# google-research/semivl

Measured on AMD Instinct MI355X. Metric: train images/sec (512^2, ViT-B/16), higher is better.
Workload: dtype f32 (fp32 in / out / accumulate everywhere; the MFMA products as split 16-bit terms with fp32 accumulation: the ViT's linears, in_proj weight gradients and fused attention and the decoder's 3x3 convolutions (tiled: forward, input and weight gradient; dilated: forward, input gradient) on fp16 x 2 ope; 1 GPU; SemiVL step, pascal N=21, vlm-vlg-aspp-s2p4-sk04-ftap-mcvitb, 512x512, bs=16/GPU labeled + 16/GPU unlabeled (BASELINE configs[1]); global_batch=32, parallelism=dp1

## Files before the change

### include/semivl_hip.h

```cpp
#ifndef SEMIVL_HIP_H_
#define SEMIVL_HIP_H_

#include <stddef.h>
#include <stdint.h>

#ifdef __cplusplus
extern "C" {
#endif

typedef void* svl_stream_t;

typedef enum svl_status {
  SVL_OK = 0,
  SVL_ERR_INVALID_ARG = -1,
  SVL_ERR_LAUNCH = -2,
  SVL_ERR_UNSUPPORTED = -3
} svl_status;

int svl_version(void);
int svl_stream_release(svl_stream_t stream);
int svl_stream_prepare(svl_stream_t stream);
int svl_stream_helper(svl_stream_t stream, void** helper);
int svl_shutdown(void);
int svl_num_stream_contexts(void);
// ... 94 lines not shown
  int64_t p_rows;
  const float* bias;
  int act;
  float* preact;
  const float* resid;
  int64_t ldr;
  int accumulate;
  int fmt;
  int p_fmt;
  const int32_t* a_sexp;
  const int32_t* b_sexp;
  const float* a_rnorm;
  const float* b_bound;
  int32_t* p_sexp;
} svl_pgemm_desc;
int64_t svl_planes_rows(int64_t rows);
int64_t svl_planes_bytes(int64_t rows, int K);
int svl_split_planes_bf16x3(const float* x, int64_t ld, int64_t k_stride, int64_t rows, int K, void* planes,
                            int64_t planes_rows, int64_t row_off, svl_stream_t stream);
int64_t svl_planes_bytes_fmt(int64_t rows, int K, int fmt);
int svl_split_planes_f16x2(const float* x, int64_t ld, int64_t k_stride, int64_t rows, int K, void* planes,
                           int64_t planes_rows, int64_t row_off, int32_t* sexp, float* rnorm, unsigned* tensor_amax,
                           svl_stream_t stream);
int svl_gemm_planes_f32(const svl_pgemm_desc* d, svl_stream_t stream);
int svl_conv3x3_wgrad_tiled_groups(int imgs, int H, int W, int Ct, int Co);
int svl_conv3x3_wgrad_tiled(const float* dy, int64_t lddy, int Co, const float* src1, int64_t ld1, int C1,
                            const float* src2, int64_t ld2, int C2, int rep, int imgs, int H, int W, float* slabs,
                            int groups, const float* gn_in, svl_stream_t stream);

int svl_reduce_slabs_f32(float* out, const float* slabs, int nslab, int64_t count, int accumulate,
                         svl_stream_t stream);


int svl_softmax_max_f32(const float* logits, int B, int N, int64_t HW, float* conf, int64_t* label,
                        svl_stream_t stream);

int svl_cutmix_f32(float* out, const float* a, const float* b, const float* box, int B, int C, int64_t HW,
                   svl_stream_t stream);
int svl_cutmix_i64(int64_t* out, const int64_t* a, const int64_t* b, const float* box, int B, int64_t HW,
                   svl_stream_t stream);

typedef struct svl_ce_desc {
  const float* logits;
  int B, N;
  int64_t HW;
  const int64_t* target;
// ... 85 lines not shown
int svl_layernorm_bwd(const float* dy, const float* x, const float* stats, const float* gamma, int64_t rows,
                      int C, const float* dx_add, float* dx, float* dgamma_part, float* dbeta_part,
                      svl_stream_t stream);
int svl_softmax_rows_fwd(float* s, int64_t rows, int cols, int64_t ld, float scale, svl_stream_t stream);
int svl_softmax_rows_bwd(float* dp, const float* p, int64_t rows, int cols, int64_t ld, float scale,
                         svl_stream_t stream);

int svl_l2norm_fwd(const float* x, int64_t rows, int C, float eps, float* y, float* inv_norm, svl_stream_t stream);
int svl_l2norm_bwd(const float* dy, const float* y, const float* inv_norm, int64_t rows, int C, float* dx,
                   svl_stream_t stream);

int64_t svl_colsum_ws_floats(int64_t rows, int C);
int svl_colsum_f32(const float* x, int64_t rows, int C, int64_t ld, float* out, int accumulate, float* ws,
                   svl_stream_t stream);

int svl_eltwise_f32(int mode, const float* a, const float* b, float* out, int64_t n, svl_stream_t stream);
int svl_chanmask_f32(const float* x, const float* mask, float scale, int64_t rows, int rows_per_img, int C,
                     float* out, svl_stream_t stream);
int svl_fill_f32(float* p, float v, int64_t n, svl_stream_t stream);
int svl_bernoulli_f32(float* p, int64_t n, float keep_prob, uint64_t seed, uint64_t offset, svl_stream_t stream);
int svl_affine_planes_f32(const float* x, int64_t planes, int C, int64_t HW, const float* k4, float* y, svl_stream_t stream);
int svl_copy2d_f32(const float* src, int64_t sgrp, int64_t src_go, int64_t src_ld, float* dst, int64_t dgrp,
                   int64_t dst_go, int64_t dst_ld, int64_t rows, int C, int accumulate, svl_stream_t stream);
int svl_permute4_f32(const float* src, float* dst, int64_t n0, int64_t n1, int64_t n2, int64_t n3, int64_t s0, int64_t s1,
                     int64_t s2, int64_t s3, svl_stream_t stream);
int svl_bound2_f32(const float* rnorm, int64_t rows, const float* bias, int64_t nbias, float* out2, svl_stream_t stream);
int svl_permute_rows_f32(const float* src, int64_t outer, int A, int B, int C, float* dst, svl_stream_t stream);

int svl_groupnorm_fwd(const float* x, int64_t ldx, const float* gamma, const float* beta, float eps, int imgs,
                      int64_t HW, int C, int G, int relu, float* y, int64_t ldy, float* stats, svl_stream_t stream);
int64_t svl_conv3x3_gn_ws_doubles(int imgs, int H, int W, int N);
int svl_conv3x3_gn_f32(const float* src1, int64_t ld1, int C1, const float* src2, int64_t ld2, int C2, int rep,
                       const float* w, int imgs, int H, int W, int N, float* out, int64_t ldo, float eps, double* ws,
                       float* stats, const float* gn_in, const void* w_planes, svl_stream_t stream);
int64_t svl_conv3x3_weight_planes_bytes(int N, int Ct);
int svl_conv3x3_weight_planes(const float* w, int N, int Ct, void* planes, svl_stream_t stream);
int svl_groupnorm_scale_shift(const float* stats, const float* gamma, const float* beta, int imgs, int C, int G, float* scsh,
                              svl_stream_t stream);
int svl_groupnorm_apply(const float* x, int64_t ldx, const float* gamma, const float* beta, int imgs, int64_t HW, int C, int G,
                        int relu, const float* stats, float* y, int64_t ldy, svl_stream_t stream);
int svl_groupnorm_bwd(const float* dy, int64_t lddy, const float* x, int64_t ldx, const float* y, int64_t ldy,
                      const float* stats, const float* gamma, const float* beta, int imgs, int64_t HW, int C, int G,
                      int relu, float* dx, int64_t lddx, float* chan_sums, svl_stream_t stream);
int64_t svl_conv3x3_gnb_ws_doubles(int imgs, int H, int W, int N);
int svl_conv3x3_dgrad_gnb_f32(const float* dy, int64_t lddy, int C1, const float* w, int imgs, int H, int W, int N, float* out,
                              int64_t ldo, int accumulate, const float* gnb_x, const float* gnb_table, const float* gnb_stats,
// ... 126 lines not shown
```

### semivl_amd/csrc/api.hip

```cpp
#include "svl_common.h"
#include <stdarg.h>

#include <map>
#include <mutex>
#include <utility>

static thread_local char g_err[512] = {0};

void svl_set_error(const char* fmt, ...) {
  va_list ap;
  va_start(ap, fmt);
  vsnprintf(g_err, sizeof(g_err), fmt, ap);
  va_end(ap);
}

extern "C" int svl_version(void) { return 604; }

extern "C" int svl_last_error(char* buf, size_t len) {
  const size_t n = strlen(g_err);
  if (buf && len > 0) {
    const size_t c = n < len - 1 ? n : len - 1;
    memcpy(buf, g_err, c);
    buf[c] = 0;
  }
  return (int)n;
}

namespace {
struct StreamCtx {
  hipStream_t aux = nullptr;
  hipEvent_t fork = nullptr, join = nullptr;
};
std::mutex g_mu;
std::map<std::pair<int, hipStream_t>, StreamCtx> g_ctx;

int stream_device(hipStream_t st, int* dev) {
  if (hipGetDevice(dev) != hipSuccess) {
    svl_set_error("hipGetDevice failed");
    return SVL_ERR_LAUNCH;
// ... 111 lines not shown
```

### semivl_amd/csrc/gemm_planes_h2.hip

```cpp
#include "gemm_planes_impl.h"
#include <stdlib.h>

int svl_planes_launch_h2(const PlanesP& p, hipStream_t st) { return launch<2>(p, st); }

namespace {

__global__ __launch_bounds__(256) void pack_planes_h2_kernel(const float* __restrict__ x, long ld, long ks, long rows, int K,
                                                             char* __restrict__ planes, long p_ks, long row_off,
                                                             int* __restrict__ sexp, float* __restrict__ rnorm,
                                                             unsigned* __restrict__ tensor_amax) {
  __shared__ float s_max[8][32];
  __shared__ double s_sq[8][32];
  __shared__ int s_e[32];
  const int tid = threadIdx.x;
  const long rb = blockIdx.x;
  const bool rowmajor = ks == 1;
  const bool fast = rowmajor && (ld & 3) == 0 && ((reinterpret_cast<uintptr_t>(x) & 15) == 0) && (K & 3) == 0;
  if (rowmajor) {
    const int row = tid >> 3, sub = tid & 7;
    const long r = rb * 32 + row;
    float amax = 0.f;
    double sq = 0.0;
    if (r < rows) {
      const float* src = x + r * ld;
      if (fast) {
        for (int k = sub * 4; k < K; k += 32) {
          const float4 f = *reinterpret_cast<const float4*>(src + k);
          amax = fmaxf(fmaxf(amax, fabsf(f.x)), fmaxf(fabsf(f.y), fmaxf(fabsf(f.z), fabsf(f.w))));
          sq += (double)f.x * f.x + (double)f.y * f.y + ((double)f.z * f.z + (double)f.w * f.w);
        }
      } else {
        for (int k = sub; k < K; k += 8) {
          const float f = src[k];
          amax = fmaxf(amax, fabsf(f));
          sq += (double)f * f;
        }
      }
    }
// ... 9 lines not shown
    float amax = 0.f;
    double sq = 0.0;
    if (r < rows)
      for (int k = part; k < K; k += 8) {
        const float f = x[r * ld + (long)k * ks];
        amax = fmaxf(amax, fabsf(f));
        sq += (double)f * f;
      }
    s_max[part][r31] = amax;
    s_sq[part][r31] = sq;
  }
  __syncthreads();
  if (tid < 32) {
    float amax = s_max[0][tid];
    double sq = s_sq[0][tid];
    if (!rowmajor)
      for (int q = 1; q < 8; ++q) { amax = fmaxf(amax, s_max[q][tid]); sq += s_sq[q][tid]; }
    const long r = rb * 32 + tid;
    const int e = r < rows ? scale_exp_of(amax) : 0;
    s_e[tid] = e;
    const long rr = row_off + rb * 32 + tid;
    sexp[rr] = e;
    if (rnorm) rnorm[rr] = r < rows ? (float)(sqrt(sq) * (1.0 + 1e-6)) : 0.f;
    if (tensor_amax && blockIdx.y == 0) {
      float m = r < rows ? amax : 0.f;
#pragma unroll
      for (int o = 16; o > 0; o >>= 1) m = fmaxf(m, __shfl_xor(m, o, 64));
      if (tid == 0 && m > 0.f) atomicMax(tensor_amax, __float_as_uint(m));
    }
  }
  __syncthreads();
  const int nkg = K >> 4;
  const int kg_lo = (int)((long)nkg * blockIdx.y / gridDim.y), kg_hi = (int)((long)nkg * (blockIdx.y + 1) / gridDim.y);
  for (int idx = kg_lo * 64 + tid; idx < kg_hi * 64; idx += 256) {
    const int r31 = idx & 31, h = (idx >> 5) & 1, kg = idx >> 6;
    const long r = rb * 32 + r31;
    float v[8];
    if (r < rows) {
      const float* src = x + r * ld + (long)(kg * 16 + 4 * h) * ks;
      if (fast) {
        const float4 f0 = *reinterpret_cast<const float4*>(src), f1 = *reinterpret_cast<const float4*>(src + 8);
        v[0] = f0.x; v[1] = f0.y; v[2] = f0.z; v[3] = f0.w; v[4] = f1.x; v[5] = f1.y; v[6] = f1.z; v[7] = f1.w;
      } else {
#pragma unroll
        for (int q = 0; q < 4; ++q) { v[q] = src[q * ks]; v[4 + q] = src[(8 + q) * ks]; }
      }
    } else {
#pragma unroll
      for (int q = 0; q < 8; ++q) v[q] = 0.f;
    }
    f16x8 h0, h1;
    split2x8(v, s_e[r31], h0, h1);
    const long rr = row_off + r;
    char* q = planes + (long)kg * p_ks + (rr >> 5) * (2 * CH) + (h * 32 + (int)(rr & 31)) * 16;
    *reinterpret_cast<f16x8*>(q) = h0;
    *reinterpret_cast<f16x8*>(q + CH) = h1;
  }
}

}

extern "C" int svl_split_planes_f16x2(const float* x, int64_t ld, int64_t k_stride, int64_t rows, int K, void* planes,
                                      int64_t planes_rows, int64_t row_off, int32_t* sexp, float* rnorm, unsigned* tensor_amax,
                                      svl_stream_t stream) {
  SVL_CHECK_ARG(x && planes && sexp && rows > 0 && K > 0 && (K & 15) == 0 && k_stride >= 1 && planes_rows >= row_off + rows &&
                    row_off >= 0 && (planes_rows & 255) == 0 && (row_off & 31) == 0,
                "svl_split_planes_f16x2: bad args (K %% 16, planes_rows %% 256, row_off %% 32 must be 0; sexp required)");
  const long blocks = (rows + 31) / 32;
  int ysplit = 1;
  if (blocks < 256) {
    ysplit = (int)(512 / blocks);
    if (ysplit > 8) ysplit = 8;
    if (ysplit > (K >> 6)) ysplit = K >> 6;
    if (ysplit < 1) ysplit = 1;
  }
  if (tensor_amax) SVL_HIP_CHECK(hipMemsetAsync(tensor_amax, 0, 4, (hipStream_t)stream));
  hipLaunchKernelGGL(pack_planes_h2_kernel, dim3((unsigned)blocks, (unsigned)ysplit), dim3(256), 0, (hipStream_t)stream, x, (long)ld,
                     (long)k_stride, (long)rows, K, (char*)planes, (long)planes_rows * 64, (long)row_off, sexp, rnorm, tensor_amax);
  SVL_LAUNCH_CHECK("svl_split_planes_f16x2");
  return SVL_OK;
}
```

### semivl_amd/csrc/norm.hip

```cpp
#include "svl_common.h"
#include "planes_split_h2.h"

namespace {

inline int grid_for(long n, int per_thread = 1) {
  long g = (n + 256L * per_thread - 1) / (256L * per_thread);
  if (g < 1) g = 1;
  if (g > 256 * 16) g = 256 * 16;
  return (int)g;
}

__device__ __forceinline__ void ln_emit_planes(const float* __restrict__ src, long r0, long rows, int C,
                                               const float* __restrict__ gamma, const float* __restrict__ beta,
                                               const float* st , char* __restrict__ planes, long p_ks) {
  const int t = threadIdx.x, r31 = t & 31, h = (t >> 5) & 1, kg0 = t >> 6;
  const long r = r0 + r31;
  const int nkg = C >> 4;
  float mean = 0.f, rstd = 0.f;
  mean = st[2 * r31]; rstd = st[2 * r31 + 1];
  for (int kg = kg0; kg < nkg; kg += 4) {
    float v[8];
    const int k = kg * 16 + 4 * h;
    if (r < rows) {
      const float4 f0 = *reinterpret_cast<const float4*>(src + r * C + k), f1 = *reinterpret_cast<const float4*>(src + r * C + k + 8);
// ... 414 lines not shown
  }
}
__global__ void chanmask_kernel(const float* __restrict__ x, const float* __restrict__ mask, float scale, long rows,
                                int rows_per_img, int C, float* __restrict__ out) {
  const long n = rows * C;
  for (long i = (long)blockIdx.x * blockDim.x + threadIdx.x; i < n; i += (long)gridDim.x * blockDim.x) {
    const long r = i / C;
    const int c = (int)(i - r * C);
    out[i] = x[i] * mask[(r / rows_per_img) * C + c] * scale;
  }
}
__global__ void copy2d_kernel(const float* __restrict__ src, long sgrp, long src_go, long src_ld,
                              float* __restrict__ dst, long dgrp, long dst_go, long dst_ld, long rows, int C,
                              int accumulate) {
  const long n = rows * C;
  for (long t = (long)blockIdx.x * blockDim.x + threadIdx.x; t < n; t += (long)gridDim.x * blockDim.x) {
    const long i = t / C;
    const int c = (int)(t - i * C);
    const float v = src[(i / sgrp) * src_go + (i % sgrp) * src_ld + c];
    float* d = dst + (i / dgrp) * dst_go + (i % dgrp) * dst_ld + c;
    *d = accumulate ? (*d + v) : v;
  }
}
__global__ void affine_planes_kernel(const float* __restrict__ x, long planes, int C, long HW, const float* __restrict__ k,
                                     float* __restrict__ y) {
  const long n = planes * HW;
  for (long i = (long)blockIdx.x * blockDim.x + threadIdx.x; i < n; i += (long)gridDim.x * blockDim.x) {
    const int c = (int)((i / HW) % C);
    y[i] = ((x[i] * k[c] + k[C + c]) - k[2 * C + c]) / k[3 * C + c];
  }
}
__global__ void bernoulli_kernel(float* p, long n, float keep, unsigned long long seed, unsigned long long offset) {
  for (long i = (long)blockIdx.x * blockDim.x + threadIdx.x; i < n; i += (long)gridDim.x * blockDim.x) {
    unsigned long long z = seed + (offset + (unsigned long long)i + 1ull) * 0x9E3779B97F4A7C15ull;
    z = (z ^ (z >> 30)) * 0xBF58476D1CE4E5B9ull;
    z = (z ^ (z >> 27)) * 0x94D049BB133111EBull;
    z ^= z >> 31;
    const float u = (float)(z >> 40) * (1.0f / 16777216.0f);
    p[i] = u < keep ? 1.f : 0.f;
  }
}
__global__ void fill_kernel(float* p, float v, long n) {
  for (long i = (long)blockIdx.x * blockDim.x + threadIdx.x; i < n; i += (long)gridDim.x * blockDim.x) p[i] = v;
}

template <int NT>
// ... 780 lines not shown
  const long total = (long)(n0 * n1 * n2 * n3);
  hipLaunchKernelGGL(permute4_kernel, dim3(grid_for(total, 4)), dim3(256), 0, (hipStream_t)stream, src, dst, (long)n1, (long)n2,
                     (long)n3, (long)s0, (long)s1, (long)s2, (long)s3, total);
  SVL_LAUNCH_CHECK("svl_permute4_f32");
  return SVL_OK;
}

extern "C" int svl_bound2_f32(const float* rnorm, int64_t rows, const float* bias, int64_t nbias, float* out2,
                              svl_stream_t stream) {
  SVL_CHECK_ARG(rnorm && rows > 0 && out2 && (!bias || nbias > 0), "svl_bound2_f32: bad args");
  hipLaunchKernelGGL(bound2_kernel, dim3(1), dim3(256), 0, (hipStream_t)stream, rnorm, (long)rows, bias, (long)nbias, out2);
  SVL_LAUNCH_CHECK("svl_bound2_f32");
  return SVL_OK;
}

extern "C" int svl_copy2d_f32(const float* src, int64_t sgrp, int64_t src_go, int64_t src_ld, float* dst, int64_t dgrp,
                              int64_t dst_go, int64_t dst_ld, int64_t rows, int C, int accumulate, svl_stream_t stream) {
  SVL_CHECK_ARG(src && dst && sgrp >= 1 && dgrp >= 1 && rows > 0 && C > 0, "svl_copy2d_f32: bad args");
  hipLaunchKernelGGL(copy2d_kernel, dim3(grid_for(rows * C, 4)), dim3(256), 0, (hipStream_t)stream, src, (long)sgrp,
                     (long)src_go, (long)src_ld, dst, (long)dgrp, (long)dst_go, (long)dst_ld, (long)rows, C, accumulate);
  SVL_LAUNCH_CHECK("svl_copy2d_f32");
  return SVL_OK;
}
```

### semivl_amd/lib.py

```python
import ctypes as C
import os
import subprocess

import torch

_HERE = os.path.dirname(os.path.abspath(__file__))
LIB_PATH = os.path.join(_HERE, "libsemivl_hip.so")
CSRC = os.path.join(_HERE, "csrc")

c_f32p = C.c_void_p
c_i64p = C.c_void_p


class Operand(C.Structure):
    _fields_ = [("ptr", C.c_void_p), ("ld", C.c_int64), ("bs_outer", C.c_int64), ("bs_inner", C.c_int64)]


class ConvGeom(C.Structure):
    _fields_ = [("H", C.c_int), ("W", C.c_int), ("Ho", C.c_int), ("Wo", C.c_int), ("stride", C.c_int),
                ("C1", C.c_int), ("C2", C.c_int), ("rep", C.c_int),
                ("KH", C.c_int), ("KW", C.c_int), ("dil", C.c_int), ("pad", C.c_int), ("sign", C.c_int),
                ("src2", C.c_void_p), ("ld2", C.c_int64), ("patch", C.c_int)]


# ... 24 lines not shown

class CeDesc(C.Structure):
    _fields_ = [("logits", C.c_void_p), ("B", C.c_int), ("N", C.c_int), ("HW", C.c_int64),
                ("target", C.c_void_p), ("use_ignore_t", C.c_int), ("conf", C.c_void_p), ("ign", C.c_void_p),
                ("conf_thresh", C.c_float), ("all_pixels", C.c_int), ("mc_target", C.c_void_p), ("partials", C.c_void_p),
                ("dlogits", C.c_void_p), ("gscale", C.c_void_p), ("img_weight", C.c_void_p)]


class CeUpDesc(C.Structure):
    _fields_ = [("logits", C.c_void_p), ("B", C.c_int), ("N", C.c_int), ("h", C.c_int), ("w", C.c_int), ("H", C.c_int),
                ("W", C.c_int), ("align_corners", C.c_int), ("target", C.c_void_p), ("use_ignore_t", C.c_int),
                ("conf", C.c_void_p), ("ign", C.c_void_p), ("conf_thresh", C.c_float), ("all_pixels", C.c_int),
                ("mc_target", C.c_void_p), ("partials", C.c_void_p), ("dlogits", C.c_void_p), ("gscale", C.c_void_p),
                ("img_weight", C.c_void_p)]


class SeqAttnDesc(C.Structure):
    _fields_ = [("groups", C.c_int), ("inner", C.c_int), ("seq", C.c_int), ("heads", C.c_int),
                ("outer_stride", C.c_int64), ("inner_stride", C.c_int64), ("seq_stride", C.c_int64),
                ("qkv", C.c_void_p), ("out", C.c_void_p), ("probs", C.c_void_p),
                ("dout", C.c_void_p), ("dqkv", C.c_void_p), ("dscores", C.c_void_p)]


_I, _L, _F, _D, _P = C.c_int, C.c_int64, C.c_float, C.c_double, C.c_void_p
SIGNATURES = {
    "svl_version": (_I, []),
    "svl_last_error": (_I, [C.c_char_p, C.c_size_t]),
    "svl_gemm_f32": (_I, [C.POINTER(GemmDesc), _P]),
    "svl_set_gemm_emulation": (_I, [_I]),
    "svl_get_gemm_emulation": (_I, []),
    "svl_set_conv_tiled": (_I, [_I]),
    "svl_planes_rows": (_L, [_L]),
    "svl_planes_bytes": (_L, [_L, _I]),
    "svl_split_planes_bf16x3": (_I, [_P, _L, _L, _L, _I, _P, _L, _L, _P]),
    "svl_planes_bytes_fmt": (_L, [_L, _I, _I]),
    "svl_split_planes_f16x2": (_I, [_P, _L, _L, _L, _I, _P, _L, _L, _P, _P, _P, _P]),
    "svl_gemm_planes_f32": (_I, [C.POINTER(PGemmDesc), _P]),
    "svl_conv3x3_wgrad_tiled_groups": (_I, [_I, _I, _I, _I, _I]),
    "svl_conv3x3_wgrad_tiled": (_I, [_P, _L, _I, _P, _L, _I, _P, _L, _I, _I, _I, _I, _I, _P, _I, _P, _P]),
    "svl_reduce_slabs_f32": (_I, [_P, _P, _I, _L, _I, _P]),
    "svl_softmax_max_f32": (_I, [_P, _I, _I, _L, _P, _P, _P]),
    "svl_cutmix_f32": (_I, [_P, _P, _P, _P, _I, _I, _L, _P]),
    "svl_cutmix_i64": (_I, [_P, _P, _P, _P, _I, _L, _P]),
    "svl_ce_num_blocks": (_L, [_I, _I, _L]),
    "svl_ce_fused_f32": (_I, [C.POINTER(CeDesc), _P]),
    "svl_ce_finalize": (_I, [_P, _L, _P, _P]),
    "svl_ce_up_num_blocks": (_L, [_I, _I, _I, _I, _I, _I, _I]),
    "svl_ce_up_fused_f32": (_I, [C.POINTER(CeUpDesc), _P]),
    "svl_softmax_max_up_f32": (_I, [_P, _I, _I, _I, _I, _I, _I, _I, _P, _P, _P]),
    "svl_semivl_gscale": (_I, [_P, _D, _F, _P, _P, _P, _P]),
    "svl_semivl_loss": (_I, [_P, _D, _F, _P, _P, _P, _P]),
    "svl_inv_count_f32": (_I, [_P, _P, _P]),
    "svl_conf_ratio_f32": (_I, [_P, _P, _I, _L, _F, _P, _P, _P]),
    "svl_conf_avg_ws_doubles": (_L, [_I]),
    "svl_conf_avg_factor": (_I, [_P, _P, _I, _L, _P, _P, _P]),
    "svl_stream_release": (_I, [_P]),
    "svl_stream_prepare": (_I, [_P]),
    "svl_stream_helper": (_I, [_P, C.POINTER(C.c_void_p)]),
    "svl_last_gemm_path": (_I, []),
# ... 13 lines not shown
    "svl_concept_max_f32": (_I, [_P, _I, _I, _L, _P, _I, _P, _P]),
    "svl_iou_hist_i64": (_I, [_P, _P, _L, _I, _I, _P, _P]),
    "svl_layernorm_fwd": (_I, [_P, _P, _P, _F, _L, _I, _P, _P, _P]),
    "svl_layernorm_fwd_planes": (_I, [_P, _P, _P, _F, _L, _I, _P, _P, _P, _L, _P]),
    "svl_layernorm_fwd_planes_f16x2": (_I, [_P, _P, _P, _F, _L, _I, _P, _P, _P, _L, _P, _P, _P]),
    "svl_layernorm_fwd_pack_f16x2": (_I, [_P, _P, _P, _F, _L, _I, _P, _P, _P, _L, _L, _P, _P, _I, _P, _P]),
    "svl_layernorm_bwd_pack_f16x2": (_I, [_P, _P, _P, _P, _L, _I, _P, _P, _P, _L, _L, _P, _P, _P, _P]),
    "svl_layernorm_bwd_parts": (_I, [_L]),
    "svl_layernorm_bwd": (_I, [_P, _P, _P, _P, _L, _I, _P, _P, _P, _P, _P]),
    "svl_softmax_rows_fwd": (_I, [_P, _L, _I, _L, _F, _P]),
    "svl_softmax_rows_bwd": (_I, [_P, _P, _L, _I, _L, _F, _P]),
    "svl_l2norm_fwd": (_I, [_P, _L, _I, _F, _P, _P, _P]),
    "svl_l2norm_bwd": (_I, [_P, _P, _P, _L, _I, _P, _P]),
    "svl_colsum_ws_floats": (_L, [_L, _I]),
    "svl_colsum_f32": (_I, [_P, _L, _I, _L, _P, _I, _P, _P]),
    "svl_eltwise_f32": (_I, [_I, _P, _P, _P, _L, _P]),
    "svl_chanmask_f32": (_I, [_P, _P, _F, _L, _I, _I, _P, _P]),
    "svl_fill_f32": (_I, [_P, _F, _L, _P]),
    "svl_affine_planes_f32": (_I, [_P, _L, _I, _L, _P, _P, _P]),
    "svl_permute_rows_f32": (_I, [_P, _L, _I, _I, _I, _P, _P]),
    "svl_permute4_f32": (_I, [_P, _P, _L, _L, _L, _L, _L, _L, _L, _L, _P]),
    "svl_bound2_f32": (_I, [_P, _L, _P, _L, _P, _P]),
    "svl_copy2d_f32": (_I, [_P, _L, _L, _L, _P, _L, _L, _L, _L, _I, _I, _P]),
    "svl_groupnorm_fwd": (_I, [_P, _L, _P, _P, _F, _I, _L, _I, _I, _I, _P, _L, _P, _P]),
    "svl_conv3x3_gn_ws_doubles": (_L, [_I, _I, _I, _I]),
    "svl_conv3x3_gn_f32": (_I, [_P, _L, _I, _P, _L, _I, _I, _P, _I, _I, _I, _I, _P, _L, _F, _P, _P, _P, _P, _P]),
    "svl_conv3x3_weight_planes_bytes": (_L, [_I, _I]),
    "svl_conv3x3_weight_planes": (_I, [_P, _I, _I, _P, _P]),
    "svl_groupnorm_scale_shift": (_I, [_P, _P, _P, _I, _I, _I, _P, _P]),
    "svl_groupnorm_apply": (_I, [_P, _L, _P, _P, _I, _L, _I, _I, _I, _P, _P, _L, _P]),
    "svl_groupnorm_bwd": (_I, [_P, _L, _P, _L, _P, _L, _P, _P, _P, _I, _L, _I, _I, _I, _P, _L, _P, _P]),
    "svl_conv3x3_gnb_ws_doubles": (_L, [_I, _I, _I, _I]),
    "svl_conv3x3_dgrad_gnb_f32": (_I, [_P, _L, _I, _P, _I, _I, _I, _I, _P, _L, _I, _P, _P, _P, _P, _P, _P, _P]),
    "svl_groupnorm_bwd_apply": (_I, [_P, _L, _P, _L, _P, _P, _P, _I, _L, _I, _I, _I, _P, _P, _L, _P]),
    "svl_bn_ws_doubles": (_L, [_L, _I]),
    "svl_bn_stats": (_I, [_P, _L, _L, _I, _P, _P, _P]),
    "svl_bn_finalize": (_I, [_P, _D, _F, _F, _P, _P, _I, _P, _P, _P]),
    "svl_bn_eval_invstd": (_I, [_P, _F, _I, _P, _P]),
    "svl_bn_apply": (_I, [_P, _L, _L, _I, _P, _P, _P, _P, _P, _L, _I, _P, _L, _P]),
    "svl_bn_bwd_reduce": (_I, [_P, _L, _P, _L, _P, _L, _P, _P, _P, _P, _L, _I, _P, _P, _P]),
    "svl_bn_bwd_apply": (_I, [_P, _L, _P, _L, _P, _L, _P, _P, _P, _P, _P, _D, _L, _I, _P, _L, _P, _L, _P]),
    "svl_maxpool3x3s2_fwd": (_I, [_P, _I, _I, _I, _I, _P, _P, _P]),
    "svl_maxpool3x3s2_bwd": (_I, [_P, _P, _I, _I, _I, _I, _P, _P]),
    "svl_aug_resample_u8": (_I, [_P, _I, _I, _I, _I, _I, _I, _I, _I, _I, _I, _I, _I, _P, _P]),
    "svl_aug_to_float": (_I, [_P, _I, C.POINTER(C.c_float), C.POINTER(C.c_float), _P, _P]),
    "svl_aug_mask_i64": (_I, [_P, _I, _I, _I, _P, _P]),
# ... 78 lines not shown
```

### semivl_amd/model/vit.py

```python
import math

import torch
import torch.nn as nn
import torch.nn.functional as F

from .. import gradsync, ops


class _MHAParams(nn.Module):
    def __init__(self, dims):
        super().__init__()
        self.in_proj_weight = nn.Parameter(torch.empty(3 * dims, dims))
        self.in_proj_bias = nn.Parameter(torch.zeros(3 * dims))
        self.out_proj = nn.Linear(dims, dims)
        nn.init.xavier_uniform_(self.in_proj_weight)
        nn.init.constant_(self.out_proj.bias, 0.)


class _AttnParams(nn.Module):
    def __init__(self, dims):
        super().__init__()
        self.attn = _MHAParams(dims)


# ... 180 lines not shown
        if dp.get("attn") is not None:
            dbr = ops.droppath_scale(dx2, dp["attn"], dp["keep"], Bn, T)
            dbrp = ops.split_planes(dbr) if pp else None
        do = ops.matmul_nn(dbrp if dbrp is not None else dbr, p["wout"])
        wout_parts.append((dbr, s["o"]))
        if D == 64 and pp and ops.attention_planes_ok() and not (s["want_v"] and dv is not None):
            dqkv, dqkv_p = ops.attention_bwd(do, s["qkv"], s["o"], s["P"], Bn, T, heads, planes=True, sets=s.get("sets"))
            dqkv_amax = dqkv_p.amax
        elif D == 64:
            dqkv = ops.attention_bwd(do, s["qkv"], s["o"], s["P"], Bn, T, heads, sets=s.get("sets"))
        else:
            dqkv = ops.vit_attention_bwd(do, s["qkv"], s["P"], Bn, T, heads, D)
        dx_res = dx2
    dvproj = None
    if s["want_v"] and dv is not None:
        dvo, dvop = ffn_ln_bwd(dv, None, s["vo"], s["st2v"], s["hv_pre"], dp.get("ffn_v"))
        dvproj = ops.matmul_nn(dvop if dvop is not None else dvo, p["wout"])
        wout_parts.append((dvo, s["vproj"]))
        dx_res = dvo if dx_res is None else ops.add(dx_res, dvo)
    if dqkv is not None and dvproj is not None:
        rows = dqkv.shape[0]
        ops.copy2d(dvproj, 0, rows, 0, E, dqkv, 2 * E, rows, 0, 3 * E, rows, E, accumulate=True)
        dvproj = dqkv_amax = None
    g["wout_parts"] = wout_parts
    if dqkv is not None:
        g["in_full"] = (dqkv, y1, dqkv_amax, s.get("y1_amax"))
        dy1 = ops.matmul_nn(dqkv_p if dqkv_p is not None else dqkv, p["win"])
    elif dvproj is not None:
        g["in_v"] = (dvproj, y1)
        dy1 = ops.matmul_nn(dvproj, p["win"][2 * E:])
    else:
        return dx_res, None, g
    if "ln1w" in want or "ln1b" in want:
        r_ = ops.layernorm_bwd(dy1, x, s["st1"], p["ln1w"], dx_add=dx_res, want_wgrad=True, planes=pp)
        g["ln1w"], g["ln1b"] = [("add", r_[1])], [("add", r_[2])]
        return r_[0], (r_[3] if pp else None), g
    if pp:
        dx_in, dx_in_p = ops.layernorm_bwd(dy1, x, s["st1"], p["ln1w"], dx_add=dx_res, planes=True)
        return dx_in, dx_in_p, g
    return ops.layernorm_bwd(dy1, x, s["st1"], p["ln1w"], dx_add=dx_res), None, g


def ffn_ln_wgrads(p, g):
    out = {}
    for key, parts in g.items():
        if key not in FFN_LN_KEYS:
# ... 554 lines not shown
            if bias.requires_grad:
                grads[id(bias)] = sink_grad(bias, lambda dst, acc: ops.colsum(df, out=dst, accumulate=acc))
        rest = [q for q in ctx.params if q is m.pos_embed or not any(q is r_ for l_ in m.layers for r_ in l_.parameters())]
        if dx is None:
            gradsync.ready(rest)
            ctx.saved = None
            return (None, None, None, None) + tuple(grads.get(id(p)) for p in ctx.params)
        if m.ln0.weight.requires_grad or m.ln0.bias.requires_grad:
            dxpre, dg_, db_ = ops.layernorm_bwd(dx, s["x_pre"], s["st0"], m.ln0.weight, want_wgrad=True)
            _sink_vectors(grads, ((m.ln0.weight, dg_), (m.ln0.bias, db_)))
        else:
            dxpre = ops.layernorm_bwd(dx, s["x_pre"], s["st0"], m.ln0.weight)
        if m.cls_token.requires_grad:
            grads[id(m.cls_token)] = sink_grad(m.cls_token, lambda dst, acc: ops.colsum(
                dxpre.view(B, T * E), out=dst.view(-1), accumulate=acc, C_=E, ld=T * E))
        wpe = m.patch_embed.projection.weight
        if wpe.requires_grad:
            dtok = ops.empty(B * NP, E, device=dev)
            ops.copy2d(dxpre, E, NP, T * E, E, dtok, 0, NP, NP * E, E, B * NP, E)
            img = s["img"]
            grads[id(wpe)] = sink_grad(wpe, lambda dst, acc: ops.matmul_tn_patch(
                dtok, img, m.patch_size, out=dst.view(E, -1), accumulate=acc))
        def pos_fn(dst, acc):
            ops.copy2d(dxpre, 0, B * T, 0, E, dst.view(-1), 0, T, 0, E, T, E, accumulate=acc)
            for b in range(1, B):
                ops.copy2d(dxpre, b * T * E, T, 0, E, dst.view(-1), 0, T, 0, E, T, E, accumulate=True)
        dpos_in = None
        if ctx.pos_is_input:
            if m.pos_embed.requires_grad:
                dpos_in = ops.empty(T, E, device=dev)
                pos_fn(dpos_in, False)
        elif m.pos_embed.requires_grad:
            grads[id(m.pos_embed)] = sink_grad(m.pos_embed, pos_fn)
        gradsync.ready(rest)
        ctx.saved = None
        return (None, None, None, dpos_in) + tuple(grads.get(id(p)) for p in ctx.params)
```

### semivl_amd/ops.py

```python
import collections
import ctypes as C
import os
import math
import weakref

import torch

from . import lib as L

A_KC, A_MC, A_CONV, A_PATCH = 0, 1, 2, 3
B_KC, B_NC, B_CONVW = 0, 1, 2
B_NC_GELU, B_NC_LN, B_PATCHT = 3, 4, 5
ACT_NONE, ACT_GELU, ACT_RELU, ACT_MUL_DGELU, ACT_MUL_DRELU = 0, 1, 2, 3, 4
OUT_STRIDED, OUT_CONVT2X, OUT_PATCH = 0, 1, 2


def _st():
    return C.c_void_p(torch.cuda.current_stream().cuda_stream)


PROFILE = None
PROFILE_SCOPE = None


# ... 231 lines not shown
        main.wait_event(ev)
        q, seq = _WG_KEEP.get(main.device.index), getattr(ev, "_svl_seq", -1)
        while q and q[0][2] <= seq:
            q.popleft()
        return
    wg = _WG.get(main.device.index)
    if wg is not None and wg.cuda_stream != main.cuda_stream:
        main.wait_stream(wg)
        _WG_KEEP[main.device.index].clear()
        for t in produced:
            if isinstance(t, torch.Tensor) and t.is_cuda:
                t.record_stream(main)


def planes_rows(rows):
    return (rows + 255) // 256 * 256


PLANES_FMT = os.environ.get("SVL_PLANES_FMT", "h2")
assert PLANES_FMT in ("h2", "b3")


class Planes:
    __slots__ = ("buf", "rows", "K", "prow", "fmt", "sexp", "rnorm", "amax", "_bd")

    def __init__(self, rows, K, device=None, buf=None, fmt=None, sexp=None, rnorm=None):
        assert K % 16 == 0
        self.fmt = fmt or PLANES_FMT
        self.rows, self.K, self.prow = rows, K, planes_rows(rows)
        dev = device if device is not None else (buf.device if buf is not None else torch.cuda.current_device())
        self._bd = self.amax = None
        if self.fmt == "h2":
            self.buf = buf if buf is not None else torch.empty(K // 16 * self.prow * 32, dtype=torch.float16, device=dev)
            self.sexp = sexp if sexp is not None else torch.empty(self.prow, dtype=torch.int32, device=dev)
            self.rnorm = rnorm
        else:
            self.buf = buf if buf is not None else torch.empty(K // 16 * self.prow * 48, dtype=torch.bfloat16, device=dev)
            self.sexp = self.rnorm = None

    @property
    def shape(self):
        return (self.rows, self.K)

    def kslice(self, k0, k1):
        assert k0 % 16 == 0 and k1 % 16 == 0 and 0 <= k0 < k1 <= self.K
        per = self.prow * (32 if self.fmt == "h2" else 48)
        return Planes(self.rows, k1 - k0, buf=self.buf[k0 // 16 * per:k1 // 16 * per], fmt=self.fmt, sexp=self.sexp,
                      rnorm=self.rnorm)


ONEPASS = not os.environ.get("SVL_NO_ONEPASS")


def split_planes(x2d, out=None, row_off=0, transpose=False, fmt=None, want_amax=False):
    assert x2d.dim() == 2 and x2d.dtype == torch.float32
    if transpose:
        K, rows = x2d.shape
        assert x2d.stride(1) == 1
        ld, ks = 1, x2d.stride(0)
    else:
        rows, K = x2d.shape
        assert x2d.stride(1) == 1
        ld, ks = x2d.stride(0), 1
    if out is None:
        out = Planes(rows, K, device=x2d.device, fmt=fmt)
# ... 36 lines not shown
        elif hasattr(v, "buf"):
            yield v.buf
            for extra in (getattr(v, "sexp", None), getattr(v, "rnorm", None)):
                if extra is not None:
                    yield extra

    def get(self):
        if self.ev is not None:
            s = torch.cuda.current_stream()
            if s.cuda_stream not in self.seen:
                s.wait_event(self.ev)
                for t in self._tensors(self.val):
                    if t.is_cuda:
                        t.record_stream(s)
                self.seen.add(s.cuda_stream)
        return self.val


def weights_changed():
    global WEIGHT_EPOCH
    WEIGHT_EPOCH += 1


def weight_planes(W, transpose=False, fmt=None):
    fmt = fmt or PLANES_FMT

    def build():
        return split_planes(W.detach(), transpose=transpose, fmt=fmt)

    base = W._base if W._base is not None else W
    if not isinstance(base, torch.nn.Parameter):
        return build()
    key = (W.data_ptr(), tuple(W.shape), W.stride(0), transpose, fmt)
    ver = (base._version, WEIGHT_EPOCH if base.requires_grad else 0)
    hit = _WPLANES.get(key)
    if hit is not None and hit[0] == ver and hit[2]() is base:
        return hit[1].get()
    pl = build()
    if len(_WPLANES) > 4096:
        _WPLANES.clear()
    _WPLANES[key] = (ver, StreamCached(pl), weakref.ref(base))
    return pl


def _out_bound(B, bias):
    key = (None if bias is None else (bias.data_ptr(), bias._version, WEIGHT_EPOCH if bias.requires_grad else 0),
           torch.cuda.current_stream().cuda_stream)
    if B._bd is None:
        B._bd = {}
    hit = B._bd.get(key)
    if hit is not None:
        return hit
    bd = torch.empty(2, dtype=torch.float32, device=B.buf.device)
    bflat = bias.detach().view(-1) if bias is not None else None
    L.check(L.load().svl_bound2_f32(_p(B.rnorm), B.rows, _p(bflat), bflat.numel() if bflat is not None else 0, _p(bd), _st()),
            "svl_bound2_f32")
    if len(B._bd) > 8:
# ... 57 lines not shown
        if planes_only and N % 16 == 0 and out is None and not accumulate:
            po = _planes_out_for(xa, M, N, resid, act)
            pgemm(xa, wb, M, N, None, po, bias, act, preact, resid)
            return po
        if out is None:
            out = empty(M, N, device=xa.buf.device)
        pgemm(xa, wb, M, N, out, None, bias, act, preact, resid, accumulate)
        return out
    assert x.stride(1) == 1 and W.is_contiguous()
    if out is None:
        out = empty(M, N, device=x.device)
    gemm(A_KC, B_KC, M, N, K, Op(x, x.stride(0)), Op(W, K), out, ldc_m=out.stride(0), bias=bias, act=act,
         resid=resid, ldr_m=resid.stride(0) if resid is not None else None, accumulate=accumulate, preact=preact)
    return out


def copy2d(src, s_off, sgrp, src_go, src_ld, dst, d_off, dgrp, dst_go, dst_ld, rows, Cc, accumulate=False):
    if accumulate:
        assert dst_go != 0 or rows <= dgrp, "copy2d: accumulating rows of different groups land on one destination (dst_go 0)"
        assert dst_ld != 0 or dgrp == 1, "copy2d: accumulating rows of one group land on one destination (dst_ld 0)"
    L.check(L.load().svl_copy2d_f32(C.c_void_p(src.data_ptr() + 4 * s_off), sgrp, src_go, src_ld,
                                    C.c_void_p(dst.data_ptr() + 4 * d_off), dgrp, dst_go, dst_ld, rows, Cc,
                                    1 if accumulate else 0, _st()), "svl_copy2d_f32")


def matmul_nn(a, b, out=None, accumulate=False, dact=ACT_NONE, z=None, planes_only=False):
    M, K = a.shape
    N = b.shape[1]
    assert b.shape[0] == K and b.stride(1) == 1
    if isinstance(a, Planes) or planes_eligible(M, N, K):
        xa = a if isinstance(a, Planes) else split_planes(a)
        wb = weight_planes(b, transpose=True, fmt=xa.fmt)
        if dact != ACT_NONE:
            assert z is not None and z.shape == (M, N) and z.stride(1) == 1 and not accumulate
        if planes_only and N % 16 == 0 and out is None and not accumulate:
            po = _planes_out_for(xa, M, N, z if dact != ACT_NONE else None, dact)
            pgemm(xa, wb, M, N, None, po, None, dact, None, z if dact != ACT_NONE else None)
            return po
        if out is None:
            out = empty(M, N, device=xa.buf.device)
        pgemm(xa, wb, M, N, out, None, None, dact, None, z if dact != ACT_NONE else None, accumulate)
        return out
    assert a.stride(1) == 1
    if out is None:
        out = empty(M, N, device=a.device)
    if dact != ACT_NONE:
# ... 1171 lines not shown
```

Baseline: 107.8 images/s.

## Batch weight-plane packing into one launch and add batched positional-grad sum

Adds a batched plane-split kernel that packs all trainable weights requested in the previous step with a single launch per 40 items whenever the weight epoch advances. Row-slice views of a parameter now reuse the whole parameter's planes instead of packing them separately. It also replaces the per-image copy2d loop for the positional-embedding gradient with one batch-sum kernel, and pre-splits dqkv planes with amax in attention backward. The aim is fewer small kernel launches and less host overhead, at the cost of more complex cache bookkeeping and eagerly packing weights that may not be used.

```diff
diff --git a/include/semivl_hip.h b/include/semivl_hip.h
--- a/include/semivl_hip.h
+++ b/include/semivl_hip.h
@@ -140,6 +140,16 @@
 int svl_split_planes_f16x2(const float* x, int64_t ld, int64_t k_stride, int64_t rows, int K, void* planes,
                            int64_t planes_rows, int64_t row_off, int32_t* sexp, float* rnorm, unsigned* tensor_amax,
                            svl_stream_t stream);
+typedef struct svl_pack_item {
+  const float* x;
+  int64_t ld, k_stride, rows;
+  int K;
+  void* planes;
+  int64_t planes_rows;
+  int32_t* sexp;
+  float* rnorm;
+} svl_pack_item;
+int svl_split_planes_f16x2_batch(const svl_pack_item* items, int n, svl_stream_t stream);
 int svl_gemm_planes_f32(const svl_pgemm_desc* d, svl_stream_t stream);
 int svl_conv3x3_wgrad_tiled_groups(int imgs, int H, int W, int Ct, int Co);
 int svl_conv3x3_wgrad_tiled(const float* dy, int64_t lddy, int Co, const float* src1, int64_t ld1, int C1,
@@ -271,6 +281,8 @@
 int svl_affine_planes_f32(const float* x, int64_t planes, int C, int64_t HW, const float* k4, float* y, svl_stream_t stream);
 int svl_copy2d_f32(const float* src, int64_t sgrp, int64_t src_go, int64_t src_ld, float* dst, int64_t dgrp,
                    int64_t dst_go, int64_t dst_ld, int64_t rows, int C, int accumulate, svl_stream_t stream);
+int svl_batch_sum_f32(const float* src, int B, int64_t n, int64_t batch_stride, float* dst, int accumulate,
+                      svl_stream_t stream);
 int svl_permute4_f32(const float* src, float* dst, int64_t n0, int64_t n1, int64_t n2, int64_t n3, int64_t s0, int64_t s1,
                      int64_t s2, int64_t s3, svl_stream_t stream);
 int svl_bound2_f32(const float* rnorm, int64_t rows, const float* bias, int64_t nbias, float* out2, svl_stream_t stream);
diff --git a/semivl_amd/csrc/api.hip b/semivl_amd/csrc/api.hip
--- a/semivl_amd/csrc/api.hip
+++ b/semivl_amd/csrc/api.hip
@@ -14,7 +14,7 @@
   va_end(ap);
 }
 
-extern "C" int svl_version(void) { return 604; }
+extern "C" int svl_version(void) { return 605; }
 
 extern "C" int svl_last_error(char* buf, size_t len) {
   const size_t n = strlen(g_err);
diff --git a/semivl_amd/csrc/gemm_planes_h2.hip b/semivl_amd/csrc/gemm_planes_h2.hip
--- a/semivl_amd/csrc/gemm_planes_h2.hip
+++ b/semivl_amd/csrc/gemm_planes_h2.hip
@@ -5,15 +5,14 @@
 
 namespace {
 
-__global__ __launch_bounds__(256) void pack_planes_h2_kernel(const float* __restrict__ x, long ld, long ks, long rows, int K,
-                                                             char* __restrict__ planes, long p_ks, long row_off,
-                                                             int* __restrict__ sexp, float* __restrict__ rnorm,
-                                                             unsigned* __restrict__ tensor_amax) {
+__device__ __forceinline__ void pack_planes_h2_block(const float* __restrict__ x, long ld, long ks, long rows, int K,
+                                                     char* __restrict__ planes, long p_ks, long row_off,
+                                                     int* __restrict__ sexp, float* __restrict__ rnorm,
+                                                     unsigned* __restrict__ tensor_amax, long rb, int ys, int nys) {
   __shared__ float s_max[8][32];
   __shared__ double s_sq[8][32];
   __shared__ int s_e[32];
   const int tid = threadIdx.x;
-  const long rb = blockIdx.x;
   const bool rowmajor = ks == 1;
   const bool fast = rowmajor && (ld & 3) == 0 && ((reinterpret_cast<uintptr_t>(x) & 15) == 0) && (K & 3) == 0;
   if (rowmajor) {
@@ -69,7 +68,7 @@
     const long rr = row_off + rb * 32 + tid;
     sexp[rr] = e;
     if (rnorm) rnorm[rr] = r < rows ? (float)(sqrt(sq) * (1.0 + 1e-6)) : 0.f;
-    if (tensor_amax && blockIdx.y == 0) {
+    if (tensor_amax && ys == 0) {
       float m = r < rows ? amax : 0.f;
 #pragma unroll
       for (int o = 16; o > 0; o >>= 1) m = fmaxf(m, __shfl_xor(m, o, 64));
@@ -78,7 +77,7 @@
   }
   __syncthreads();
   const int nkg = K >> 4;
-  const int kg_lo = (int)((long)nkg * blockIdx.y / gridDim.y), kg_hi = (int)((long)nkg * (blockIdx.y + 1) / gridDim.y);
+  const int kg_lo = (int)((long)nkg * ys / nys), kg_hi = (int)((long)nkg * (ys + 1) / nys);
   for (int idx = kg_lo * 64 + tid; idx < kg_hi * 64; idx += 256) {
     const int r31 = idx & 31, h = (idx >> 5) & 1, kg = idx >> 6;
     const long r = rb * 32 + r31;
@@ -105,6 +104,51 @@
   }
 }
 
+__global__ __launch_bounds__(256) void pack_planes_h2_kernel(const float* __restrict__ x, long ld, long ks, long rows, int K,
+                                                             char* __restrict__ planes, long p_ks, long row_off,
+                                                             int* __restrict__ sexp, float* __restrict__ rnorm,
+                                                             unsigned* __restrict__ tensor_amax) {
+  pack_planes_h2_block(x, ld, ks, rows, K, planes, p_ks, row_off, sexp, rnorm, tensor_amax, blockIdx.x, (int)blockIdx.y,
+                       (int)gridDim.y);
+}
+
+constexpr int PACK_BATCH = 40;
+struct PackBatchItem {
+  const float* x;
+  long ld, ks, rows;
+  char* planes;
+  long p_ks;
+  int* sexp;
+  float* rnorm;
+  int K, nys;
+};
+struct PackBatchP {
+  PackBatchItem it[PACK_BATCH];
+  int start[PACK_BATCH + 1];
+  int n;
+};
+static_assert(sizeof(PackBatchP) <= 4096, "the table must fit the kernel-argument segment");
+
+__global__ __launch_bounds__(256) void pack_planes_h2_batch_kernel(const PackBatchP p) {
+  int i = 0;
+  while (i + 1 < p.n && (int)blockIdx.x >= p.start[i + 1]) ++i;
+  const int local = (int)blockIdx.x - p.start[i];
+  const int nrb = (int)((p.it[i].rows + 31) >> 5);
+  pack_planes_h2_block(p.it[i].x, p.it[i].ld, p.it[i].ks, p.it[i].rows, p.it[i].K, p.it[i].planes, p.it[i].p_ks, 0,
+                       p.it[i].sexp, p.it[i].rnorm, nullptr, local % nrb, local / nrb, p.it[i].nys);
+}
+
+int pack_ysplit(long blocks, int K) {
+  int ysplit = 1;
+  if (blocks < 256) {
+    ysplit = (int)(512 / blocks);
+    if (ysplit > 8) ysplit = 8;
+    if (ysplit > (K >> 6)) ysplit = K >> 6;
+    if (ysplit < 1) ysplit = 1;
+  }
+  return ysplit;
+}
+
 }
 
 extern "C" int svl_split_planes_f16x2(const float* x, int64_t ld, int64_t k_stride, int64_t rows, int K, void* planes,
@@ -114,16 +158,43 @@
                     row_off >= 0 && (planes_rows & 255) == 0 && (row_off & 31) == 0,
                 "svl_split_planes_f16x2: bad args (K %% 16, planes_rows %% 256, row_off %% 32 must be 0; sexp required)");
   const long blocks = (rows + 31) / 32;
-  int ysplit = 1;
-  if (blocks < 256) {
-    ysplit = (int)(512 / blocks);
-    if (ysplit > 8) ysplit = 8;
-    if (ysplit > (K >> 6)) ysplit = K >> 6;
-    if (ysplit < 1) ysplit = 1;
-  }
+  const int ysplit = pack_ysplit(blocks, K);
   if (tensor_amax) SVL_HIP_CHECK(hipMemsetAsync(tensor_amax, 0, 4, (hipStream_t)stream));
   hipLaunchKernelGGL(pack_planes_h2_kernel, dim3((unsigned)blocks, (unsigned)ysplit), dim3(256), 0, (hipStream_t)stream, x, (long)ld,
                      (long)k_stride, (long)rows, K, (char*)planes, (long)planes_rows * 64, (long)row_off, sexp, rnorm, tensor_amax);
   SVL_LAUNCH_CHECK("svl_split_planes_f16x2");
   return SVL_OK;
 }
+
+extern "C" int svl_split_planes_f16x2_batch(const svl_pack_item* items, int n, svl_stream_t stream) {
+  SVL_CHECK_ARG(items && n > 0, "svl_split_planes_f16x2_batch: bad args");
+  for (int i = 0; i < n; ++i) {
+    const svl_pack_item& t = items[i];
+    SVL_CHECK_ARG(t.x && t.planes && t.sexp && t.rows > 0 && t.rows < (1L << 30) && t.K > 0 && (t.K & 15) == 0 && t.k_stride >= 1 &&
+                      t.planes_rows >= t.rows && (t.planes_rows & 255) == 0,
+                  "svl_split_planes_f16x2_batch: bad item %d (K %% 16, planes_rows %% 256 must be 0; sexp required)", i);
+  }
+  for (int i0 = 0; i0 < n;) {
+    PackBatchP p;
+    memset(&p, 0, sizeof(p));
+    long total = 0;
+    int m = 0;
+    for (; m < PACK_BATCH && i0 + m < n; ++m) {
+      const svl_pack_item& t = items[i0 + m];
+      const long blocks = (t.rows + 31) / 32;
+      const int ys = pack_ysplit(blocks, t.K);
+      if (m > 0 && total + blocks * ys > (1L << 30)) break;
+      PackBatchItem& d = p.it[m];
+      d.x = t.x; d.ld = (long)t.ld; d.ks = (long)t.k_stride; d.rows = (long)t.rows; d.K = t.K; d.nys = ys;
+      d.planes = static_cast<char*>(t.planes); d.p_ks = (long)t.planes_rows * 64; d.sexp = t.sexp; d.rnorm = t.rnorm;
+      p.start[m] = (int)total;
+      total += blocks * ys;
+    }
+    p.start[m] = (int)total;
+    p.n = m;
+    hipLaunchKernelGGL(pack_planes_h2_batch_kernel, dim3((unsigned)total), dim3(256), 0, (hipStream_t)stream, p);
+    SVL_LAUNCH_CHECK("svl_split_planes_f16x2_batch");
+    i0 += m;
+  }
+  return SVL_OK;
+}
diff --git a/semivl_amd/csrc/norm.hip b/semivl_amd/csrc/norm.hip
--- a/semivl_amd/csrc/norm.hip
+++ b/semivl_amd/csrc/norm.hip
@@ -460,6 +460,29 @@
     *d = accumulate ? (*d + v) : v;
   }
 }
+__global__ __launch_bounds__(256) void batch_sum_kernel(const float* __restrict__ src, int B, long n, long bs,
+                                                        float* __restrict__ dst, int accumulate, int vec) {
+  const long gid = (long)blockIdx.x * blockDim.x + threadIdx.x, gsz = (long)gridDim.x * blockDim.x;
+  const long nv = vec ? n >> 2 : 0;
+  for (long i = gid; i < nv; i += gsz) {
+    const float4* s = reinterpret_cast<const float4*>(src) + i;
+    float4 a = accumulate ? reinterpret_cast<const float4*>(dst)[i] : *s;
+#pragma unroll 8
+    for (int b = accumulate ? 0 : 1; b < B; ++b) {
+      const float4 x = s[(long)b * (bs >> 2)];
+      a.x = __fadd_rn(a.x, x.x);
+      a.y = __fadd_rn(a.y, x.y);
+      a.z = __fadd_rn(a.z, x.z);
+      a.w = __fadd_rn(a.w, x.w);
+    }
+    reinterpret_cast<float4*>(dst)[i] = a;
+  }
+  for (long i = nv * 4 + gid; i < n; i += gsz) {
+    float a = accumulate ? dst[i] : src[i];
+    for (int b = accumulate ? 0 : 1; b < B; ++b) a = __fadd_rn(a, src[(long)b * bs + i]);
+    dst[i] = a;
+  }
+}
 __global__ void affine_planes_kernel(const float* __restrict__ x, long planes, int C, long HW, const float* __restrict__ k,
                                      float* __restrict__ y) {
   const long n = planes * HW;
@@ -1286,3 +1309,13 @@
   SVL_LAUNCH_CHECK("svl_copy2d_f32");
   return SVL_OK;
 }
+
+extern "C" int svl_batch_sum_f32(const float* src, int B, int64_t n, int64_t batch_stride, float* dst, int accumulate,
+                                 svl_stream_t stream) {
+  SVL_CHECK_ARG(src && dst && B >= 1 && n > 0 && (B == 1 || batch_stride >= 0), "svl_batch_sum_f32: bad args");
+  const int vec = ((reinterpret_cast<uintptr_t>(src) | reinterpret_cast<uintptr_t>(dst)) & 15) == 0 && (batch_stride & 3) == 0;
+  hipLaunchKernelGGL(batch_sum_kernel, dim3(grid_for(vec ? (n + 3) / 4 : n)), dim3(256), 0, (hipStream_t)stream, src, B, (long)n,
+                     (long)batch_stride, dst, accumulate, vec);
+  SVL_LAUNCH_CHECK("svl_batch_sum_f32");
+  return SVL_OK;
+}
diff --git a/semivl_amd/lib.py b/semivl_amd/lib.py
--- a/semivl_amd/lib.py
+++ b/semivl_amd/lib.py
@@ -70,6 +70,11 @@
                 ("dout", C.c_void_p), ("dqkv", C.c_void_p), ("dscores", C.c_void_p)]
 
 
+class PackItem(C.Structure):
+    _fields_ = [("x", C.c_void_p), ("ld", C.c_int64), ("k_stride", C.c_int64), ("rows", C.c_int64), ("K", C.c_int),
+                ("planes", C.c_void_p), ("planes_rows", C.c_int64), ("sexp", C.c_void_p), ("rnorm", C.c_void_p)]
+
+
 _I, _L, _F, _D, _P = C.c_int, C.c_int64, C.c_float, C.c_double, C.c_void_p
 SIGNATURES = {
     "svl_version": (_I, []),
@@ -83,6 +88,7 @@
     "svl_split_planes_bf16x3": (_I, [_P, _L, _L, _L, _I, _P, _L, _L, _P]),
     "svl_planes_bytes_fmt": (_L, [_L, _I, _I]),
     "svl_split_planes_f16x2": (_I, [_P, _L, _L, _L, _I, _P, _L, _L, _P, _P, _P, _P]),
+    "svl_split_planes_f16x2_batch": (_I, [C.POINTER(PackItem), _I, _P]),
     "svl_gemm_planes_f32": (_I, [C.POINTER(PGemmDesc), _P]),
     "svl_conv3x3_wgrad_tiled_groups": (_I, [_I, _I, _I, _I, _I]),
     "svl_conv3x3_wgrad_tiled": (_I, [_P, _L, _I, _P, _L, _I, _P, _L, _I, _I, _I, _I, _I, _P, _I, _P, _P]),
@@ -142,6 +148,7 @@
     "svl_permute4_f32": (_I, [_P, _P, _L, _L, _L, _L, _L, _L, _L, _L, _P]),
     "svl_bound2_f32": (_I, [_P, _L, _P, _L, _P, _P]),
     "svl_copy2d_f32": (_I, [_P, _L, _L, _L, _P, _L, _L, _L, _L, _I, _I, _P]),
+    "svl_batch_sum_f32": (_I, [_P, _I, _L, _L, _P, _I, _P]),
     "svl_groupnorm_fwd": (_I, [_P, _L, _P, _P, _F, _I, _L, _I, _I, _I, _P, _L, _P, _P]),
     "svl_conv3x3_gn_ws_doubles": (_L, [_I, _I, _I, _I]),
     "svl_conv3x3_gn_f32": (_I, [_P, _L, _I, _P, _L, _I, _I, _P, _I, _I, _I, _I, _P, _L, _F, _P, _P, _P, _P, _P]),
diff --git a/semivl_amd/model/vit.py b/semivl_amd/model/vit.py
--- a/semivl_amd/model/vit.py
+++ b/semivl_amd/model/vit.py
@@ -226,6 +226,9 @@
         rows = dqkv.shape[0]
         ops.copy2d(dvproj, 0, rows, 0, E, dqkv, 2 * E, rows, 0, 3 * E, rows, E, accumulate=True)
         dvproj = dqkv_amax = None
+        if ops.planes_eligible(rows, E, 3 * E):
+            dqkv_p = ops.split_planes(dqkv, want_amax=True)
+            dqkv_amax = dqkv_p.amax
     g["wout_parts"] = wout_parts
     if dqkv is not None:
         g["in_full"] = (dqkv, y1, dqkv_amax, s.get("y1_amax"))
@@ -826,6 +829,9 @@
             grads[id(wpe)] = sink_grad(wpe, lambda dst, acc: ops.matmul_tn_patch(
                 dtok, img, m.patch_size, out=dst.view(E, -1), accumulate=acc))
         def pos_fn(dst, acc):
+            if ops.BATCH_SUM:
+                ops.batch_sum(dxpre.view(-1), B, T * E, T * E, dst.view(-1), accumulate=acc)
+                return
             ops.copy2d(dxpre, 0, B * T, 0, E, dst.view(-1), 0, T, 0, E, T, E, accumulate=acc)
             for b in range(1, B):
                 ops.copy2d(dxpre, b * T * E, T, 0, E, dst.view(-1), 0, T, 0, E, T, E, accumulate=True)
diff --git a/semivl_amd/ops.py b/semivl_amd/ops.py
--- a/semivl_amd/ops.py
+++ b/semivl_amd/ops.py
@@ -277,14 +277,14 @@
 
 
 class Planes:
-    __slots__ = ("buf", "rows", "K", "prow", "fmt", "sexp", "rnorm", "amax", "_bd")
+    __slots__ = ("buf", "rows", "K", "prow", "fmt", "sexp", "rnorm", "amax", "_bd", "_views")
 
     def __init__(self, rows, K, device=None, buf=None, fmt=None, sexp=None, rnorm=None):
         assert K % 16 == 0
         self.fmt = fmt or PLANES_FMT
         self.rows, self.K, self.prow = rows, K, planes_rows(rows)
         dev = device if device is not None else (buf.device if buf is not None else torch.cuda.current_device())
-        self._bd = self.amax = None
+        self._bd = self.amax = self._views = None
         if self.fmt == "h2":
             self.buf = buf if buf is not None else torch.empty(K // 16 * self.prow * 32, dtype=torch.float16, device=dev)
             self.sexp = sexp if sexp is not None else torch.empty(self.prow, dtype=torch.int32, device=dev)
@@ -296,6 +296,13 @@
     @property
     def shape(self):
         return (self.rows, self.K)
+
+    def rowslice(self, r0):
+        assert self.fmt == "h2" and r0 % 256 == 0 and 0 <= r0 < self.rows
+        v = Planes(self.rows - r0, self.K, buf=self.buf[r0 * 32:], fmt=self.fmt, sexp=self.sexp[r0:],
+                   rnorm=None if self.rnorm is None else self.rnorm[r0:])
+        v.prow = self.prow
+        return v
 
     def kslice(self, k0, k1):
         assert k0 % 16 == 0 and k1 % 16 == 0 and 0 <= k0 < k1 <= self.K
@@ -378,6 +385,54 @@
     WEIGHT_EPOCH += 1
 
 
+WEIGHT_BATCH = not os.environ.get("SVL_NO_WEIGHT_BATCH")
+_WASKED = ({}, {})
+_WASKED_EPOCH = 0
+
+
+def split_planes_batch(items):
+    arr = (L.PackItem * len(items))()
+    out = []
+    for it, (x2d, transpose) in zip(arr, items):
+        assert x2d.dim() == 2 and x2d.dtype == torch.float32 and x2d.stride(1) == 1
+        if transpose:
+            (K, rows), ld, ks = x2d.shape, 1, x2d.stride(0)
+        else:
+            (rows, K), ld, ks = x2d.shape, x2d.stride(0), 1
+        pl = Planes(rows, K, device=x2d.device, fmt="h2")
+        pl.rnorm = torch.empty(pl.prow, dtype=torch.float32, device=x2d.device)
+        it.x, it.ld, it.k_stride, it.rows, it.K = x2d.data_ptr(), ld, ks, rows, K
+        it.planes, it.planes_rows, it.sexp, it.rnorm = pl.buf.data_ptr(), pl.prow, pl.sexp.data_ptr(), pl.rnorm.data_ptr()
+        out.append(pl)
+    L.check(L.load().svl_split_planes_f16x2_batch(arr, len(items), _st()), "svl_split_planes_f16x2_batch")
+    return out
+
+
+def _rebuild_asked(first_key, first_W, first_transpose):
+    global _WASKED, _WASKED_EPOCH
+    first_base = first_W._base if first_W._base is not None else first_W
+    _WASKED = (_WASKED[1], {first_key: weakref.ref(first_base)})
+    _WASKED_EPOCH = WEIGHT_EPOCH
+    todo = [(first_key, first_W.detach(), first_transpose, first_base)]
+    for key, ref in _WASKED[0].items():
+        base = ref()
+        if key == first_key or base is None or not base.requires_grad or not base.is_contiguous():
+            continue
+        ptr, shape, ld, transpose, _ = key
+        off = (ptr - base.data_ptr()) // 4
+        if off < 0 or base.data_ptr() + 4 * off != ptr or off + (shape[0] - 1) * ld + shape[1] > base.numel():
+            continue
+        x2d = base.detach().as_strided(shape, (ld, 1), base.storage_offset() + off)
+        assert x2d.data_ptr() == ptr
+        todo.append((key, x2d, transpose, base))
+    planes = split_planes_batch([(x, tr) for _, x, tr, _ in todo])
+    if len(_WPLANES) + len(todo) > 4096:
+        _WPLANES.clear()
+    for (key, _, _, base), pl in zip(todo, planes):
+        _WPLANES[key] = ((base._version, WEIGHT_EPOCH), StreamCached(pl), weakref.ref(base))
+    return planes[0]
+
+
 def weight_planes(W, transpose=False, fmt=None):
     fmt = fmt or PLANES_FMT
 
@@ -387,8 +442,24 @@
     base = W._base if W._base is not None else W
     if not isinstance(base, torch.nn.Parameter):
         return build()
+    if (WEIGHT_BATCH and fmt == "h2" and not transpose and W is not base and W.dim() == 2 and base.dim() == 2
+            and W.stride() == base.stride() and W.shape[1] == base.shape[1]):
+        r0, rem = divmod((W.data_ptr() - base.data_ptr()) // 4, base.stride(0))
+        if rem == 0 and r0 > 0 and r0 % 256 == 0 and r0 + W.shape[0] == base.shape[0]:
+            whole = weight_planes(base, fmt=fmt)
+            if whole._views is None:
+                whole._views = {}
+            v = whole._views.get(r0)
+            if v is None:
+                v = whole._views[r0] = whole.rowslice(r0)
+            return v
     key = (W.data_ptr(), tuple(W.shape), W.stride(0), transpose, fmt)
     ver = (base._version, WEIGHT_EPOCH if base.requires_grad else 0)
+    batched = WEIGHT_BATCH and fmt == "h2" and base.requires_grad and W.is_cuda and W.dim() == 2 and W.stride(1) == 1
+    if batched:
+        if _WASKED_EPOCH != WEIGHT_EPOCH:
+            return _rebuild_asked(key, W, transpose)
+        _WASKED[1][key] = weakref.ref(base)
     hit = _WPLANES.get(key)
     if hit is not None and hit[0] == ver and hit[2]() is base:
         return hit[1].get()
@@ -492,6 +563,16 @@
     L.check(L.load().svl_copy2d_f32(C.c_void_p(src.data_ptr() + 4 * s_off), sgrp, src_go, src_ld,
                                     C.c_void_p(dst.data_ptr() + 4 * d_off), dgrp, dst_go, dst_ld, rows, Cc,
                                     1 if accumulate else 0, _st()), "svl_copy2d_f32")
+
+
+BATCH_SUM = not os.environ.get("SVL_NO_BATCH_SUM")
+
+
+def batch_sum(src, B, n, batch_stride, dst, accumulate=False):
+    assert src.dtype == dst.dtype == torch.float32 and dst.numel() >= n and src.numel() >= (B - 1) * batch_stride + n
+    L.check(L.load().svl_batch_sum_f32(_p(src), B, n, batch_stride, _p(dst), 1 if accumulate else 0, _st()),
+            "svl_batch_sum_f32")
+    return dst
 
 
 def matmul_nn(a, b, out=None, accumulate=False, dact=ACT_NONE, z=None, planes_only=False):
```

Result: no change. 108.5 images/s (median of 6 runs) (+0.6%).
